# SunYangtian/UniGeo

Measured on AMD Instinct MI355X. Metric: frames/sec (384x512, 25-frame clip, 25 denoise steps), higher is better.
Workload: dtype fp16; 1 GPU; DepthCrafter SVD-UNet fp16, 25-step Euler, 25-frame 384x512 clips (BASELINE configs[1]); CLIP + VAE enc/dec + depth post-proc inside the timed region; one clip per ug_dc_run call, one call at a time (SURVEY 8d; reference eval.py:33-39); frames=25, height=384, width=512, denoise_steps=25, parallelism=clip-sharded x1, RCCL all_gather of depth, clips_in_flight_per_gpu=1, lanes=1

## Files before the change

### unigeo_amd/_lib.py

```python
import ctypes as C
import dataclasses
import json
import os
import warnings

import numpy as np

_HERE = os.path.dirname(os.path.abspath(__file__))
LIB_PATH = os.environ.get("UG_LIB_PATH") or os.path.join(_HERE, "csrc", "libunigeo_hip.so")

EXPORTS = [
    "ug_unet_config_default", "ug_vae_config_default", "ug_clip_config_default",
    "ug_create", "ug_destroy", "ug_last_error", "ug_workspace_peak",
    "ug_load_tensor", "ug_bind_unet", "ug_bind_vae", "ug_bind_clip",
    "ug_dc_set_inputs", "ug_dc_run", "ug_dc_run_windows", "ug_dc_get_outputs", "ug_dc_device_ptrs", "ug_dc_set_trace", "ug_dc_set_guidance", "ug_unet_forward_pair", "ug_dc_set_inputs_ex", "ug_dc_get_noise", "ug_op_philox_u32", "ug_op_randn", "ug_op_u8_to_frames", "ug_set_vae_encode_fp32", "ug_set_concurrency", "ug_set_coscheduled", "ug_set_fp8_linears", "ug_op_linear_mx8", "ug_set_ff_fused", "ug_op_ff", "ug_op_ln_ff", "ug_bench_ff", "ug_bench_flash", "ug_tune_flash", "ug_tune_ff",
    "ug_eval_depth", "ug_eval_normal", "ug_depth_eval_opts_default", "ug_eval_depth_ex", "ug_eval_depth_global", "ug_op_masked_median", "ug_eval_depth_l1_info", "ug_op_l1_fit", "ug_clip_embed", "ug_vae_encode", "ug_vae_decode", "ug_unet_forward", "ug_normals_from_depth",
    "ug_op_linear", "ug_op_conv", "ug_op_conv_gn", "ug_op_groupnorm", "ug_op_layernorm", "ug_op_flash_attn",
    "ug_op_temporal_attn", "ug_op_attention_generic", "ug_op_flash_attn_dh", "ug_op_euler_step", "ug_op_flash_cross_attn", "ug_op_temporal_attn_nv",
    "ug_op_groupnorm_ex", "ug_op_layernorm_ex",
    "ug_op_split_pair", "ug_op_gn32_pair", "ug_op_conv_wide", "ug_op_attn_wide",
    "ug_bind_stablenormal", "ug_sn_run", "ug_sn_unet_forward", "ug_sn_dino", "ug_sn_vae_decode", "ug_sn_vae_encode", "ug_resize_bilinear",
    "ug_pcd_opts_default", "ug_pcd_world_points", "ug_eval_pcd", "ug_op_pcd_nn", "ug_op_pcd_select", "ug_op_pcd_knn_normals", "ug_eval_pcd_fps", "ug_op_pcd_fps",
    "ug_eval_pcd_ex", "ug_op_pcd_nn_grid", "ug_op_pcd_knn_normals_grid",
    "ug_pointmap_opts_default", "ug_pointmap_focal", "ug_pointmap_poses",
    "ug_vis_depth_range", "ug_vis_panels", "ug_prep_resize_frames", "ug_prep_gt", "ug_prep_gt_ex",
    "ug_register_opts_default", "ug_prep_register_depth",
    "ug_profile_begin", "ug_profile_begin_shapes", "ug_profile_end", "ug_bench_gemm", "ug_bench_groupnorm", "ug_bench_mfma_peak", "ug_tune_force",
]


class UNetConfigC(C.Structure):
    _fields_ = [("in_channels", C.c_int), ("out_channels", C.c_int), ("num_levels", C.c_int),
                ("block_out_channels", C.c_int * 8), ("num_attention_heads", C.c_int * 8),
                ("down_has_attn", C.c_int * 8),
                ("layers_per_block", C.c_int), ("cross_attention_dim", C.c_int),
                ("addition_time_embed_dim", C.c_int), ("projection_class_embeddings_input_dim", C.c_int),
                ("norm_groups", C.c_int),
                ("eps_cross_attn_blocks", C.c_float), ("eps_plain_down_block", C.c_float),
                ("eps_mid_block", C.c_float), ("eps_up_blocks", C.c_float)]


class VAEConfigC(C.Structure):
# ... 100 lines not shown
    _set_argtypes(lib, {"ug_eval_pcd_fps": [vp, vp, vp, vp, C.c_long, C.c_long, C.POINTER(PcdOptsC), vp, vp, vp, vp, vp],
                        "ug_op_pcd_fps": [vp, vp, C.c_long, C.c_long, vp, vp]})
    _set_argtypes(lib, {"ug_eval_pcd_ex": [vp, vp, vp, vp, C.c_long, vp, C.c_long, C.POINTER(PcdOptsC), ip, vp, vp, vp, vp, vp, vp],
                        "ug_op_pcd_nn_grid": [vp, vp, C.c_long, vp, C.c_long, vp, vp, vp, vp],
                        "ug_op_pcd_knn_normals_grid": [vp, vp, C.c_long, ip, vp, vp, vp]})
    _set_argtypes(lib, {"ug_pointmap_opts_default": [C.POINTER(PointmapOptsC)],
                        "ug_pointmap_focal": [vp, vp, ip, ip, C.c_double, C.c_double, vp],
                        "ug_pointmap_poses": [vp, vp, vp, ip, ip, ip, C.c_double, C.c_double, C.c_double, C.POINTER(PointmapOptsC), vp, vp, vp, vp]})
    if hasattr(lib, "ug_pointmap_opts_default"):
        lib.ug_pointmap_opts_default.restype = None
    _set_argtypes(lib, {"ug_vis_depth_range": [vp, vp, C.c_long, vp],
                        "ug_vis_panels": [vp, vp, vp, vp, ip, ip, ip, ip, C.c_float, C.c_float, vp, vp, ip, vp]})
    _set_argtypes(lib, {"ug_prep_resize_frames": [vp, vp, ip, ip, ip, ip, ip, vp, vp, ip, vp, vp, ip, vp],
                        "ug_prep_gt": [vp, vp, C.c_float, vp, vp, vp, ip, ip, ip, vp, ip, vp, ip, C.c_float, vp, vp, vp, vp, vp],
                        "ug_prep_gt_ex": [vp, vp, C.c_float, vp, vp, vp, ip, ip, ip, vp, ip, vp, ip, C.c_float, vp, vp, vp, vp, vp, C.c_uint]})
    _set_argtypes(lib, {"ug_register_opts_default": [C.POINTER(RegisterOptsC)],
                        "ug_prep_register_depth": [vp, vp, ip, ip, ip, C.POINTER(RegisterOptsC), vp]})
    lib.ug_clip_embed.argtypes = [vp, vp, ip, ip, ip, vp]
    lib.ug_vae_encode.argtypes = [vp, vp, ip, ip, ip, vp]
    lib.ug_vae_decode.argtypes = [vp, vp, ip, ip, ip, vp]
    lib.ug_unet_forward.argtypes = [vp, vp, ip, ip, ip, C.c_float, vp, vp]
    lib.ug_normals_from_depth.argtypes = [vp, vp, vp, ip, ip, ip, vp]
    lib.ug_op_linear.argtypes = [vp, vp, ip, ip, vp, ip, vp, vp, C.c_float, C.c_float, ip, ip, vp]
    lib.ug_op_conv.argtypes = [vp, vp, ip, vp, ip, ip, ip, ip, vp, vp, ip, ip, ip, ip, ip, ip, ip, vp]
    lib.ug_op_groupnorm.argtypes = [vp, vp, ip, vp, ip, ip, ip, ip, C.c_float, ip, ip, vp, vp, vp]
    lib.ug_op_conv_gn.argtypes = [vp, vp, ip, ip, ip, ip, vp, vp, vp, ip, ip, ip, ip, C.c_float, ip, vp, vp, vp, vp, vp, vp]
    lib.ug_op_layernorm.argtypes = [vp, vp, ip, ip, C.c_float, vp, vp, vp, ip, vp, vp]
    lib.ug_op_flash_attn.argtypes = [vp, vp, ip, ip, ip, vp]
    lib.ug_op_temporal_attn.argtypes = [vp, vp, ip, ip, ip, vp]
    lib.ug_op_attention_generic.argtypes = [vp, vp, ip, ip, ip, ip, vp]
# ... 55 lines not shown
    c = VAEConfigC()
    c.in_channels, c.out_channels, c.latent_channels = cfg.in_channels, cfg.out_channels, cfg.latent_channels
    c.num_levels = len(cfg.block_out_channels)
    _fill8(c.block_out_channels, cfg.block_out_channels)
    c.layers_per_block, c.norm_groups, c.scaling_factor = cfg.layers_per_block, cfg.norm_groups, cfg.scaling_factor
    return c


def _clip_c(cfg):
    c = CLIPConfigC()
    c.hidden_size, c.intermediate_size = cfg.hidden_size, cfg.intermediate_size
    c.num_hidden_layers, c.num_attention_heads = cfg.num_hidden_layers, cfg.num_attention_heads
    c.image_size, c.patch_size, c.layer_norm_eps = cfg.image_size, cfg.patch_size, cfg.layer_norm_eps
    c.projection_dim = getattr(cfg, "projection_dim", 0)
    return c


class Engine:

    def __init__(self, device_id=0, workspace_bytes=2 << 30, persist_bytes=1 << 30):
        self.lib = load_library()
        self.ctx = self.lib.ug_create(int(device_id), int(workspace_bytes), int(persist_bytes))
        if not self.ctx:
            raise RuntimeError("ug_create failed: " + self.lib.ug_last_error(None).decode())
        self.device_id = device_id
        self.l1_info = None
        self._l1_warned = False

    def close(self):
        if getattr(self, "ctx", None):
# ... 762 lines not shown
        cv = conv or {}
        self._ck(self.lib.ug_bench_gemm(self.ctx, M, N, K, int(conv is not None), cv.get("T", 0), cv.get("H", 0), cv.get("W", 0),
                                        cv.get("C0", 0), cv.get("C1", 0), cv.get("kt", 1), cv.get("k", 1), cv.get("stride", 1),
                                        cv.get("ups", 1), cfg, split, iters, _ptr(out)))
        Mr, Kr = float(out[3]), float(out[4])
        return float(out[0]), 2.0 * Mr * N * Kr / (out[0] * 1e-3) / 1e12, int(out[1]), int(out[2])

    def bench_mfma_peak(self, iters=20000):
        out = np.zeros(1, np.float32)
        self._ck(self.lib.ug_bench_mfma_peak(self.ctx, int(iters), _ptr(out)))
        return float(out[0])

    def tune_force(self, cfg=-1, split=-1):
        self._ck(self.lib.ug_tune_force(self.ctx, int(cfg), int(split)))

    def bench_groupnorm(self, C0, C1, T, HW, temporal, mode, iters=20):
        out = np.zeros(1, np.float32)
        self._ck(self.lib.ug_bench_groupnorm(self.ctx, C0, C1, T, HW, int(temporal), mode, iters, _ptr(out)))
        return float(out[0])

    def profile_begin(self, shapes=False):
        self._ck((self.lib.ug_profile_begin_shapes if shapes else self.lib.ug_profile_begin)(self.ctx))

    def profile_end(self):
        prof = json.loads(self.lib.ug_profile_end(self.ctx).decode())
        self.last_profile_order = prof.pop("__order__", None)
        return prof

    def workspace_peak(self):
        return int(self.lib.ug_workspace_peak(self.ctx))
# ... 1 lines not shown
```

### unigeo_amd/csrc/common.h

```cpp
#pragma once
#include <hip/hip_runtime.h>
#include <hip/hip_fp16.h>
#include <stdint.h>
#include <stdio.h>
#include <stdexcept>
#include <string>

typedef _Float16 f16;
typedef _Float16 f16x2 __attribute__((ext_vector_type(2)));
typedef _Float16 f16x4 __attribute__((ext_vector_type(4)));
typedef _Float16 f16x8 __attribute__((ext_vector_type(8)));
typedef float f32x4 __attribute__((ext_vector_type(4)));
typedef float f32x16 __attribute__((ext_vector_type(16)));

#define UG_CHECK(expr)                                                                        \
  do {                                                                                        \
    hipError_t _e = (expr);                                                                   \
    if (_e != hipSuccess)                                                                     \
      throw std::runtime_error(std::string(#expr) + " failed: " + hipGetErrorString(_e) +    \
                               " at " + __FILE__ + ":" + std::to_string(__LINE__));           \
  } while (0)

#define UG_REQUIRE(cond, msg)                                                                 \
  do {                                                                                        \
    if (!(cond))                                                                              \
      throw std::runtime_error(std::string("requirement failed: ") + #cond + " : " + (msg) + \
                               " at " + __FILE__ + ":" + std::to_string(__LINE__));           \
  } while (0)

static inline int cdiv(long a, long b) { return (int)((a + b - 1) / b); }
static inline int ug_dev_slot() { int d = 0; (void)hipGetDevice(&d); return d & 31; }

enum { UG_ACT_NONE = 0, UG_ACT_SILU = 1, UG_ACT_GELU = 2 };
enum { UG_F_GEGLU = 1, UG_F_OUT_F32 = 2, UG_F_NOXCD = 4, UG_F_PRIO = 8 ,
       UG_F_XCDROUND = 32 ,
       UG_F_R1_F32 = 16  };

struct GemmP {
  const f16* A0; const f16* A1;
  int C0, C1;
  int M, N, K;
  int conv;
  int T, Hi, Wi, Ho, Wo;
  int ups, stride, pad_t, pad_l;
  int kt, ky, kx;
  const f16* W; long ldw;
  const f16* bias; const f16* bias2;
  const f16* R1; long ldr1; float c1;
  const f16* R2; long ldr2; float c2;
  float c0;
  void* Out; long ldo;
// ... 13 lines not shown
  int group_m;
  int halo_tw, halo_lg;
  int tune_cfg_p1, tune_split_p1, tune_knobs;
  float2* stat_part; int stat_hw;
};
struct GemmTune { int cfg = -1, split = -1, knobs = 0; };
static inline void gemm_apply_tune(GemmP& p, const GemmTune& t) { p.tune_cfg_p1 = t.cfg + 1; p.tune_split_p1 = t.split + 1; p.tune_knobs = t.knobs; }
void launch_gemm_mx8(const GemmP& p, hipStream_t s);
void launch_quant_mx8(const f16* x, long ldx, long M, int K, unsigned char* q, unsigned* scales, long ld_s, hipStream_t s);
void launch_gemm(const GemmP& p, int batch, hipStream_t s, int* stat_rb = nullptr);
bool gemm_stream_supported(const GemmP& p, int batch);
void launch_gemm_stream(const GemmP& p, hipStream_t s);
bool conv_halo_supported(const GemmP& p, int batch, int bm, int bn);
void launch_conv_halo(const GemmP& p, int bm, int bn, hipStream_t s);
void gemm_plan(const GemmP& p, int batch, int* cfg_out, int* split_out);

struct FFusedP {
  const f16* X; const f16* W1; const f16* b1; const f16* W2; const f16* b2;
  const f16* R1; const f16* R2; float c0, c1, c2;
  f16* Out; int M, C; const f16* zero;
  const f16* ln_g; const f16* ln_b; float ln_eps; const f16* addvec; int rows_per_vec;
  int variant;
};
bool ff_fused_supported(int C);
void launch_ff_fused(const FFusedP& p, hipStream_t s);

struct GroupNormP {
  const f16* X0; const f16* X1; int C0, C1;
  int T, HW, G; float eps; int temporal; int silu;
  const f16* gamma; const f16* beta;
// ... 227 lines not shown
```

### unigeo_amd/csrc/kernels/gemm.hip

```cpp
#include "../common.h"
#include <algorithm>

#include "gemm_common.h"

template <int BM, int BN, int BK, int NST, int WMW, int WNW> struct GemmOcc {
  static constexpr int lds = NST * (BM + BN) * BK * 2;
  static constexpr int wg_lds = (160 * 1024) / lds;
  static constexpr int wg = wg_lds < 1 ? 1 : (wg_lds > 4 ? 4 : wg_lds);
  static constexpr int wps_raw = wg * WMW * WNW / 4;
  static constexpr int wps = wps_raw < 1 ? 1 : (wps_raw > 4 ? 4 : wps_raw);
};

#ifdef UG_GEMM_TRACE
#define UG_STAMP(slot)                                                                                   \
  do {                                                                                                   \
    if (traced && fi >= 8 && fi < 32) {                                                                  \
      unsigned long long c_;                                                                             \
      asm volatile("s_memtime %0\n\ts_waitcnt lgkmcnt(0)" : "=s"(c_)::"memory");                         \
      if (lane == 0) tr_lds[(fi - 8) * 5 + (slot)] = (unsigned)c_;                                       \
    }                                                                                                    \
  } while (0)
#else
#define UG_STAMP(slot) do {} while (0)
#endif
// ... 21 lines not shown
  const int wm = wave / WNW, wn = wave % WNW;
  if (NWAVE == 8 && wave >= 4 && ((BM == 256 && BN == 256) || (p.flags & UG_F_PRIO))) __builtin_amdgcn_s_setprio(1);
  const int ntn = (p.N + BN - 1) / BN, ntm = (p.M + BM - 1) / BM;
  const int ntiles = ntm * ntn;

  const int bz = blockIdx.z;
  const int bo = bz / p.nb_inner, bi = bz - bo * p.nb_inner;
  const f16* A0 = p.A0 + bo * p.sA_o + bi * p.sA_i;
  const f16* Wb = p.W + bo * p.sW_o + bi * p.sW_i;
  const long out_off = bo * p.sO_o + bi * p.sO_i;

  const int pc = lane % CPR;
  const int lrow = lane / CPR;
  const int Cin = p.C0 + p.C1;

  const int nk_all = (p.K + BK - 1) / BK;
  int kt_lo = 0, kt_hi = nk_all;
  if (p.splitk > 1) {
    const int per = (nk_all + p.splitk - 1) / p.splitk;
    kt_lo = min(nk_all, (int)blockIdx.y * per);
    kt_hi = min(nk_all, kt_lo + per);
  }
  const int nk = max(kt_hi - kt_lo, 1);

  const int nwg = gridDim.x, w = blockIdx.x;
  const TileWalk tw = tile_walk(p.flags, ntiles, nwg, w);
  const int my_tiles = tw.count;
  const int total_it = my_tiles * nk;

  int a_lc[AI]; bool a_ok[AI]; const f16* a_ptr[AI]; int a_t[AI], a_y[AI], a_x[AI];
  int a_pix[AI]; unsigned a_mask[AI];
  const bool fastconv = CONV && UNI;
  int a_par[AI];
  int b_lc[BI]; const f16* b_ptr[BI]; bool b_ok[BI];
  unsigned a_off[AI], a_off1[AI], b_off[BI];
  const int cshift = CONV ? ((p.kt >> 1) * p.Hi + p.pad_t) * p.Wi + p.pad_l : 0;
  __amdgpu_buffer_rsrc_t rA0, rA1, rW;
  if (BUFA) {
    rA0 = __builtin_amdgcn_make_buffer_rsrc((void*)(A0 - (long)cshift * p.C0), 0, (int)SENT, 0x00020000);
    rA1 = __builtin_amdgcn_make_buffer_rsrc((void*)((CONV && p.A1) ? p.A1 - (long)cshift * p.C1 : A0), 0, (int)SENT, 0x00020000);
    rW = __builtin_amdgcn_make_buffer_rsrc((void*)Wb, 0, (int)SENT, 0x00020000);
  }
// ... 252 lines not shown
    if (traced && fi == 40) {
      __builtin_amdgcn_s_waitcnt(0);
      for (int i = lane; i < 24 * 5; i += 64) ((unsigned*)p.trace)[(wave == 4 ? 24 * 5 : 0) + i] = tr_lds[i];
    }
#endif
    if (++cp_ks != nk) continue;
    cp_ks = 0;
    const int ti = cp_ti++;

    drain = true;
    const int tile = tw.first + ti * tw.step;
    { int etm, etn; tile_coord_p(p, tile, ntm, ntn, etm, etn);
      if constexpr (ST) tile_epilogue_stats<MT, NT, WTM, WTN>(p, acc, etm * BM, etn * BN, wm, wn, lane, etm * WMW + wm);
      else if constexpr (BM * BN < 65536) {
        if (lean_epi == 1) tile_epilogue_lean<MT, NT, WTM, WTN, false>(p, acc, etm * BM, etn * BN, wm, wn, lane, out_off, nullptr);
        else if constexpr (NT == 4 && !CONV) { if (lean_epi == 2) tile_epilogue_geglu_lean<MT, NT, WTM, WTN>(p, acc, etm * BM, etn * BN, wm, wn, lane, out_off); else tile_epilogue<MT, NT, WTM, WTN>(p, acc, etm * BM, etn * BN, wm, wn, lane, out_off); }
        else tile_epilogue<MT, NT, WTM, WTN>(p, acc, etm * BM, etn * BN, wm, wn, lane, out_off);
      } else if constexpr (NT == 4 && !CONV) { if (lean_epi == 2) tile_epilogue_geglu_lean<MT, NT, WTM, WTN>(p, acc, etm * BM, etn * BN, wm, wn, lane, out_off); else tile_epilogue<MT, NT, WTM, WTN>(p, acc, etm * BM, etn * BN, wm, wn, lane, out_off); }
      else tile_epilogue<MT, NT, WTM, WTN>(p, acc, etm * BM, etn * BN, wm, wn, lane, out_off); }
  }
}

template <int BM, int BN, int NST, int WMW, int WNW, bool CONV, bool ST = false>
__global__ __launch_bounds__(512, 2) void gemm_ldr_kernel(const GemmP p) {
  constexpr int BK = 64;
  static_assert(WMW * WNW == 8, "two waves per SIMD");
  constexpr unsigned SENT = 0x80000000u;
  constexpr int WTM = BM / WMW, WTN = BN / WNW;
  constexpr int MT = WTM / 16, NT = WTN / 16;
  constexpr int WID = 4 * NT;
  constexpr int AI = BM / 64, BI = BN / 64;
  constexpr int LA = 2 * AI, LB = 2 * BI;
  constexpr int STAGE = (BM + BN) * BK;
  static_assert(AI >= 1 && BI >= 1 && NST >= 2 && NST <= 3, "tile / ring");
// ... 4 lines not shown
  const int wave = __builtin_amdgcn_readfirstlane(tid >> 6);
  const int wm = wave / WNW, wn = wave % WNW;
  const bool loader = wave >= 4;
  const int ntn = (p.N + BN - 1) / BN, ntm = (p.M + BM - 1) / BM;
  const int ntiles = ntm * ntn;

  const int bz = blockIdx.z;
  const int bo = bz / p.nb_inner, bi = bz - bo * p.nb_inner;
  const f16* A0 = p.A0 + bo * p.sA_o + bi * p.sA_i;
  const f16* Wb = p.W + bo * p.sW_o + bi * p.sW_i;
  const long out_off = bo * p.sO_o + bi * p.sO_i;

  const int pc = lane & 7, lrow = lane >> 3;
  const int Cin = p.C0 + p.C1;

  const int nk_all = (p.K + BK - 1) / BK;
  int kt_lo = 0, kt_hi = nk_all;
  if (p.splitk > 1) {
    const int per = (nk_all + p.splitk - 1) / p.splitk;
    kt_lo = min(nk_all, (int)blockIdx.y * per);
    kt_hi = min(nk_all, kt_lo + per);
  }
  const int nk = max(kt_hi - kt_lo, 1);

  const int nwg = gridDim.x, w = blockIdx.x;
  const TileWalk tw = tile_walk(p.flags, ntiles, nwg, w);
  const int my_tiles = tw.count;
  const int total_it = my_tiles * nk;

  unsigned a_st[LA], b_off[LB];
  const int lc16_0 = (pc ^ ((0 + (lrow >> 1)) & 7)) * 16, lc16_1 = (pc ^ ((4 + (lrow >> 1)) & 7)) * 16;
  const int cshift = CONV ? ((p.kt >> 1) * p.Hi + p.pad_t) * p.Wi + p.pad_l : 0;
  const __amdgpu_buffer_rsrc_t rA0 = __builtin_amdgcn_make_buffer_rsrc((void*)(A0 - (long)cshift * p.C0), 0, (int)SENT, 0x00020000);
  const __amdgpu_buffer_rsrc_t rA1 =
      __builtin_amdgcn_make_buffer_rsrc((void*)((CONV && p.A1) ? p.A1 - (long)cshift * p.C1 : A0), 0, (int)SENT, 0x00020000);
  const __amdgpu_buffer_rsrc_t rW = __builtin_amdgcn_make_buffer_rsrc((void*)Wb, 0, (int)SENT, 0x00020000);

  auto setup_tile = [&](int tile) {
    int tm, tn; tile_coord_p(p, tile, ntm, ntn, tm, tn);
    const int m0 = tm * BM, n0 = tn * BN;
#pragma unroll
    for (int l = 0; l < LA; ++l) {
// ... 144 lines not shown
    }
#ifdef UG_GEMM_TRACE
    if (traced && fi == 40) {
      __builtin_amdgcn_s_waitcnt(0);
      for (int i = lane; i < 24 * 5; i += 64) ((unsigned*)p.trace)[(wave == 4 ? 24 * 5 : 0) + i] = tr_lds[i];
    }
#endif
    if (++cp_ks != nk) continue;
    cp_ks = 0;
    const int tile = tw.first + (cp_ti++) * tw.step;
    drain = true;
    { int etm, etn; tile_coord_p(p, tile, ntm, ntn, etm, etn);
      if constexpr (ST) tile_epilogue_stats<MT, NT, WTM, WTN>(p, acc, etm * BM, etn * BN, wm, wn, lane, etm * WMW + wm);
      else if constexpr (BM * BN < 65536) {
        if (lean_epi == 1) tile_epilogue_lean<MT, NT, WTM, WTN, false>(p, acc, etm * BM, etn * BN, wm, wn, lane, out_off, nullptr);
        else if constexpr (NT == 4 && !CONV) { if (lean_epi == 2) tile_epilogue_geglu_lean<MT, NT, WTM, WTN>(p, acc, etm * BM, etn * BN, wm, wn, lane, out_off); else tile_epilogue<MT, NT, WTM, WTN>(p, acc, etm * BM, etn * BN, wm, wn, lane, out_off); }
        else tile_epilogue<MT, NT, WTM, WTN>(p, acc, etm * BM, etn * BN, wm, wn, lane, out_off);
      } else if constexpr (NT == 4 && !CONV) { if (lean_epi == 2) tile_epilogue_geglu_lean<MT, NT, WTM, WTN>(p, acc, etm * BM, etn * BN, wm, wn, lane, out_off); else tile_epilogue<MT, NT, WTM, WTN>(p, acc, etm * BM, etn * BN, wm, wn, lane, out_off); }
      else tile_epilogue<MT, NT, WTM, WTN>(p, acc, etm * BM, etn * BN, wm, wn, lane, out_off); }
  }
}

static bool gemm_can_bufa(const GemmP& p, int BK, bool packed) {
  const long lim = (1L << 31) - 64;
  if ((long)p.N * p.ldw * 2 >= lim) return false;
  if (p.conv) {
    const bool kc_ok = p.kchunk || p.kt * p.ky * p.kx == 1 || (p.C0 + p.C1) == BK;
    const bool uni = kc_ok && ((p.C0 + p.C1) % BK) == 0 && (p.C0 % BK) == 0 && p.kt * p.ky * p.kx <= (packed ? 9 : 32);
    const long px = (long)p.T * p.Hi * p.Wi + ((long)(p.kt >> 1) * p.Hi + p.pad_t) * p.Wi + p.pad_l + 1;
    return uni && p.ups == 1 && px * p.C0 * 2 < lim && px * p.C1 * 2 < lim && (!packed || px < (1L << 23));
  }
  return p.K % BK == 0 && (long)p.M * p.C0 * 2 < lim;
}

// ... 17 lines not shown
  constexpr int STAGE = (BM + BN) * BK;
  extern __shared__ __attribute__((aligned(16))) f16 smem[];

  const int tid = threadIdx.x, lane = tid & 63;
  const int wave = __builtin_amdgcn_readfirstlane(tid >> 6);
  const bool producer = wave >= NCW;
  const int ntn = (p.N + BN - 1) / BN, ntm = (p.M + BM - 1) / BM;
  const int ntiles = ntm * ntn;

  const int bz = blockIdx.z;
  const int bo = bz / p.nb_inner, bi = bz - bo * p.nb_inner;
  const f16* A0 = p.A0 + bo * p.sA_o + bi * p.sA_i;
  const f16* Wb = p.W + bo * p.sW_o + bi * p.sW_i;
  const long out_off = bo * p.sO_o + bi * p.sO_i;

  const int nk_all = (p.K + BK - 1) / BK;
  int kt_lo = 0, kt_hi = nk_all;
  if (p.splitk > 1) {
    const int per = (nk_all + p.splitk - 1) / p.splitk;
    kt_lo = min(nk_all, (int)blockIdx.y * per);
    kt_hi = min(nk_all, kt_lo + per);
  }
  const int nk = max(kt_hi - kt_lo, 1);

  const int nwg = gridDim.x, w = blockIdx.x;
  const TileWalk tw = tile_walk(p.flags, ntiles, nwg, w);
  const int my_tiles = tw.count;
  const int total_it = my_tiles * nk;

  if (producer) {
    const int pw = wave - NCW;
    const int pc = lane & 7, lrow = lane >> 3;
    const int Cin = p.C0 + p.C1;
    const int lc16_0 = (pc ^ ((0 + (lrow >> 1)) & 7)) * 16, lc16_1 = (pc ^ ((4 + (lrow >> 1)) & 7)) * 16;
    const int cshift = CONV ? ((p.kt >> 1) * p.Hi + p.pad_t) * p.Wi + p.pad_l : 0;
    const __amdgpu_buffer_rsrc_t rA0 = __builtin_amdgcn_make_buffer_rsrc((void*)(A0 - (long)cshift * p.C0), 0, (int)SENT, 0x00020000);
    const __amdgpu_buffer_rsrc_t rA1 =
        __builtin_amdgcn_make_buffer_rsrc((void*)((CONV && p.A1) ? p.A1 - (long)cshift * p.C1 : A0), 0, (int)SENT, 0x00020000);
    const __amdgpu_buffer_rsrc_t rW = __builtin_amdgcn_make_buffer_rsrc((void*)Wb, 0, (int)SENT, 0x00020000);
    unsigned a_st[LA], b_off[LB];
    int ld_ti = 0, ld_ks = 0, ld_slot = 0;
    int u_it = 0, u_iy = 0, u_ix = 0, u_cb = 0;
// ... 184 lines not shown
    }
    UG_STAMP(1);
    asm volatile("s_waitcnt lgkmcnt(0)" ::: "memory");
    UG_STAMP(2);
    __builtin_amdgcn_s_barrier();
    asm volatile("" ::: "memory");
    UG_STAMP(3);
    if (++cp_ks == nk) {
      cp_ks = 0;
      const int tile = tw.first + (cp_ti++) * tw.step;
      { int etm, etn; tile_coord_p(p, tile, ntm, ntn, etm, etn);
        if constexpr (ST) tile_epilogue_stats<MT, NT, WTM, WTN>(p, acc, etm * BM, etn * BN, wm, wn, lane, etm * WMW + wm);
        else if (PREK && do_pre) {
          if (lean) tile_epilogue_lean<MT, NT, WTM, WTN, PREK>(p, acc, etm * BM, etn * BN, wm, wn, lane, out_off, &pre);
          else if constexpr (NT == 4) { if (lean_geglu) tile_epilogue_geglu_lean<MT, NT, WTM, WTN>(p, acc, etm * BM, etn * BN, wm, wn, lane, out_off);
            else tile_epilogue<MT, NT, WTM, WTN, PREK>(p, acc, etm * BM, etn * BN, wm, wn, lane, out_off, &pre); }
          else tile_epilogue<MT, NT, WTM, WTN, PREK>(p, acc, etm * BM, etn * BN, wm, wn, lane, out_off, &pre);
        } else if constexpr (PREK) {
          tile_epilogue<MT, NT, WTM, WTN>(p, acc, etm * BM, etn * BN, wm, wn, lane, out_off);
        } else {
          if (lean) tile_epilogue_lean<MT, NT, WTM, WTN, false>(p, acc, etm * BM, etn * BN, wm, wn, lane, out_off, nullptr);
          else if constexpr (NT == 4) { if (lean_geglu) tile_epilogue_geglu_lean<MT, NT, WTM, WTN>(p, acc, etm * BM, etn * BN, wm, wn, lane, out_off);
            else tile_epilogue<MT, NT, WTM, WTN>(p, acc, etm * BM, etn * BN, wm, wn, lane, out_off); }
          else tile_epilogue<MT, NT, WTM, WTN>(p, acc, etm * BM, etn * BN, wm, wn, lane, out_off);
        } }
    }
#ifdef UG_GEMM_TRACE
    if (traced && fi == 40) {
      __builtin_amdgcn_s_waitcnt(0);
      for (int i = lane; i < 24 * 5; i += 64) ((unsigned*)p.trace)[(wave == 4 ? 24 * 5 : 0) + i] = tr_lds[i];
    }
#endif
  }
}

template <int BN, int WMW, int WNW, int BM = 256>
static void launch_ws(const GemmP& p, int batch, hipStream_t s) {
  const int ntiles = cdiv(p.M, BM) * cdiv(p.N, BN);
#ifdef UG_GEMM_TRACE
  const size_t lds = ws_nst(BM, BN) * (BM + BN) * 64 * sizeof(f16) + 2048;
#else
  const size_t lds = ws_nst(BM, BN) * (BM + BN) * 64 * sizeof(f16);
#endif
  static bool attr[32] = {};
  bool& at = attr[ug_dev_slot()];
  if (!at) {
    UG_CHECK(hipFuncSetAttribute((const void*)gemm_ws_kernel<BM, BN, WMW, WNW, true>, hipFuncAttributeMaxDynamicSharedMemorySize, (int)lds));
    UG_CHECK(hipFuncSetAttribute((const void*)gemm_ws_kernel<BM, BN, WMW, WNW, false>, hipFuncAttributeMaxDynamicSharedMemorySize, (int)lds));
    at = true;
  }
  const int split = p.splitk > 1 ? p.splitk : 1;
  int gx = std::max(8, 256 / (split * batch));
  gx = (gx / 8) * 8;
  gx = std::min(gx, ntiles);
  dim3 grid(gx, split, batch);
  if (p.stat_part) {
    if constexpr (BN == 128) {
      UG_REQUIRE(p.conv, "producer / consumer kernel: epilogue statistics for convolutions only");
      static bool attrs[32] = {};
      bool& ats = attrs[ug_dev_slot()];
      if (!ats) { UG_CHECK(hipFuncSetAttribute((const void*)gemm_ws_kernel<BM, BN, WMW, WNW, true, true>, hipFuncAttributeMaxDynamicSharedMemorySize, (int)lds)); ats = true; }
      hipLaunchKernelGGL((gemm_ws_kernel<BM, BN, WMW, WNW, true, true>), grid, dim3((WMW * WNW + 4) * 64), lds, s, p);
      return;
    } else UG_REQUIRE(false, "producer / consumer kernel: epilogue statistics on 128-column tiles only");
  }
  if (p.conv) hipLaunchKernelGGL((gemm_ws_kernel<BM, BN, WMW, WNW, true>), grid, dim3((WMW * WNW + 4) * 64), lds, s, p);
  else hipLaunchKernelGGL((gemm_ws_kernel<BM, BN, WMW, WNW, false>), grid, dim3((WMW * WNW + 4) * 64), lds, s, p);
}

template <int BM, int BN, int NST, int WMW, int WNW>
static void launch_ldr(const GemmP& p, int batch, hipStream_t s) {
  UG_REQUIRE(p.m_off == 0, "row-split launches need the producer / consumer kernel");
  const int ntiles = cdiv(p.M, BM) * cdiv(p.N, BN);
#ifdef UG_GEMM_TRACE
  const size_t lds = (size_t)NST * (BM + BN) * 64 * sizeof(f16) + 1024;
#else
  const size_t lds = (size_t)NST * (BM + BN) * 64 * sizeof(f16);
#endif
  static bool attr[32] = {};
  bool& at = attr[ug_dev_slot()];
  if (!at) {
    UG_CHECK(hipFuncSetAttribute((const void*)gemm_ldr_kernel<BM, BN, NST, WMW, WNW, true>, hipFuncAttributeMaxDynamicSharedMemorySize, (int)lds));
    UG_CHECK(hipFuncSetAttribute((const void*)gemm_ldr_kernel<BM, BN, NST, WMW, WNW, false>, hipFuncAttributeMaxDynamicSharedMemorySize, (int)lds));
    at = true;
  }
  const int per_cu = (160 * 1024) / (int)lds < 1 ? 1 : std::min(2, (160 * 1024) / (int)lds);
  const int split = p.splitk > 1 ? p.splitk : 1;
  int gx = std::max(8, (per_cu * 256) / (split * batch));
  gx = (gx / 8) * 8;
  gx = std::min(gx, ntiles);
  dim3 grid(gx, split, batch);
  if (p.stat_part) {
    if constexpr (BM == 256 && BN == 256) {
      UG_REQUIRE(p.conv, "loader kernel: epilogue statistics for convolutions only");
      static bool attrs[32] = {};
      bool& ats = attrs[ug_dev_slot()];
      if (!ats) { UG_CHECK(hipFuncSetAttribute((const void*)gemm_ldr_kernel<BM, BN, NST, WMW, WNW, true, true>, hipFuncAttributeMaxDynamicSharedMemorySize, (int)lds)); ats = true; }
      hipLaunchKernelGGL((gemm_ldr_kernel<BM, BN, NST, WMW, WNW, true, true>), grid, dim3(512), lds, s, p);
      return;
    } else UG_REQUIRE(false, "loader kernel: epilogue statistics on the 256 x 256 tile only");
  }
  if (p.conv) hipLaunchKernelGGL((gemm_ldr_kernel<BM, BN, NST, WMW, WNW, true>), grid, dim3(512), lds, s, p);
  else hipLaunchKernelGGL((gemm_ldr_kernel<BM, BN, NST, WMW, WNW, false>), grid, dim3(512), lds, s, p);
}

__global__ __launch_bounds__(256) void splitk_epilogue(const GemmP p) {
// ... 24 lines not shown
    if (p.act == UG_ACT_SILU) {
#pragma unroll
      for (int q = 0; q < 8; ++q) v[q] = silu_f(v[q]);
    } else if (p.act == UG_ACT_GELU) {
#pragma unroll
      for (int q = 0; q < 8; ++q) v[q] = gelu_f(v[q]);
    }
    f16x8 h;
#pragma unroll
    for (int q = 0; q < 8; ++q) h[q] = (f16)v[q];
    *(f16x8*)((f16*)p.Out + m * p.ldo + n) = h;
  }
}

template <int BM, int BN, int BK, int NST, int WMW, int WNW, bool CONV, bool UNI, bool BUFA = false, bool ST = false>
static void launch_t(const GemmP& p, int batch, hipStream_t s) {
  const int ntiles = cdiv(p.M, BM) * cdiv(p.N, BN);
#ifdef UG_GEMM_TRACE
  const size_t lds = (size_t)NST * (BM + BN) * BK * sizeof(f16) + 1024;
#else
  const size_t lds = (size_t)NST * (BM + BN) * BK * sizeof(f16);
#endif
  auto kern = gemm_kernel<BM, BN, BK, NST, WMW, WNW, CONV, UNI, BUFA, false, ST>;
  static bool attr[32] = {};
  bool& at = attr[ug_dev_slot()];
  if (!at) {
    if (lds > 64 * 1024) UG_CHECK(hipFuncSetAttribute((const void*)kern, hipFuncAttributeMaxDynamicSharedMemorySize, (int)lds));
    at = true;
  }
  const int per_cu = GemmOcc<BM, BN, BK, NST, WMW, WNW>::wg;
  const int split = p.splitk > 1 ? p.splitk : 1;
  const int cap = std::max(8, (per_cu * 256) / (split * batch));
  int gx = (cap / 8) * 8;
  gx = std::min(gx, ntiles);
  if (gx < ntiles && cap >= ntiles) gx = ntiles;
  if (p.tune_knobs & 1) gx = ntiles;
  dim3 grid(gx, split, batch);
  hipLaunchKernelGGL(kern, grid, dim3(WMW * WNW * 64), lds, s, p);
}

template <int BM, int BN, int BK, int NST, int WMW, int WNW>
static void launch_mode(const GemmP& p, int batch, hipStream_t s) {
  UG_REQUIRE(p.m_off == 0, "row-split launches need the producer / consumer kernel");
  const long lim = (1L << 31) - 64;
  const bool bufw = (long)p.N * p.ldw * 2 < lim && !(p.tune_knobs & 4);
  if (p.conv) {
    const bool kc_ok = p.kchunk || p.kt * p.ky * p.kx == 1 || (p.C0 + p.C1) == BK;
    const bool uni = kc_ok && ((p.C0 + p.C1) % BK) == 0 && (p.C0 % BK) == 0 && p.kt * p.ky * p.kx <= 32;
    const long px = (long)p.T * p.Hi * p.Wi + ((long)(p.kt >> 1) * p.Hi + p.pad_t) * p.Wi + p.pad_l + 1;
    const bool bufa = bufw && uni && p.ups == 1 && px * p.C0 * 2 < lim && px * p.C1 * 2 < lim;
    if (p.stat_part) {
      if constexpr ((BM == 256 && BN == 64 && NST == 2 && WMW == 4) || (BM == 256 && BN == 128 && NST == 3 && WMW == 2)) { UG_REQUIRE(uni && bufa, "statistics epilogue: buffer-addressed im2col only"); launch_t<BM, BN, BK, NST, WMW, WNW, true, true, true, true>(p, batch, s); return; }
// ... 351 lines not shown
```

### unigeo_amd/csrc/kernels/gemm_common.h

```cpp
#pragma once
#include "../common.h"
#include <type_traits>

typedef const __attribute__((address_space(1))) void* gptr_t;
typedef __attribute__((address_space(3))) void* lptr_t;

__device__ __forceinline__ float erf_as(float x) {
  const float ax = fabsf(x);
  const float t = __frcp_rn(1.0f + 0.3275911f * ax);
  const float y = ((((1.061405429f * t - 1.453152027f) * t + 1.421413741f) * t - 0.284496736f) * t + 0.254829592f) * t;
  const float r = 1.0f - y * __expf(-ax * ax);
  return copysignf(r, x);
}
__device__ __forceinline__ float gelu_f(float x) { return 0.5f * x * (1.0f + erf_as(x * 0.70710678118654752f)); }
__device__ __forceinline__ float silu_f(float x) { return x * __builtin_amdgcn_rcpf(1.0f + __expf(-x)); }

typedef float f32x2 __attribute__((ext_vector_type(2)));
__device__ __forceinline__ f32x2 geglu2(f32x2 h, f32x2 g) {
  const f32x2 ag = {__builtin_fabsf(g.x), __builtin_fabsf(g.y)};
  const f32x2 u = ag * 0.23164189f + 1.0f;
  const f32x2 t = {__builtin_amdgcn_rcpf(u.x), __builtin_amdgcn_rcpf(u.y)};
  f32x2 y = t * 0.5307027145f - 0.7265760135f;
  y = y * t + 0.7107068705f;
  y = y * t - 0.142248368f;
// ... 24 lines not shown
  tile_coord(tile, ntm, ntn, p.group_m, tm, tn);
  if (p.tm_T) { const int q = tm / p.tm_T; tm = (tm - q * p.tm_T) * p.tm_nb + q; }
}

struct TileWalk { int first, step, count; };
__device__ __forceinline__ TileWalk tile_walk(int flags, int ntiles, int nwg, int w) {
  TileWalk t;
  if (nwg % 8 != 0 || (flags & UG_F_NOXCD)) { t.first = w; t.step = nwg; t.count = (ntiles - w + nwg - 1) / nwg; return t; }
  const int x = w & 7, j = w >> 3, npx = nwg >> 3;
  if (flags & UG_F_XCDROUND) { t.first = x * npx + j; t.step = nwg; t.count = (ntiles - t.first + nwg - 1) / nwg; return t; }
  const int lo = (int)(((long)x * ntiles) >> 3), hi = (int)(((long)(x + 1) * ntiles) >> 3);
  t.first = lo + j; t.step = npx; t.count = max(0, (hi - lo - j + npx - 1) / npx);
  return t;
}

template <int N> struct HVec;
template <> struct HVec<8> { typedef f16x8 type; };
template <> struct HVec<4> { typedef f16x4 type; };

template <int MT, int NT> struct EpiPre {
  static constexpr int WID = 4 * NT, CH = (WID % 8 == 0) ? 8 : 4, NV = WID / CH;
  typedef typename HVec<CH>::type hvec;
  hvec b1[NV], b2[NV];
  hvec r1[MT][NV];
};
template <int MT, int NT, int WTM, int WTN>
__device__ __forceinline__ void epi_pre_cols(const GemmP& p, int n0, int wn, int lane, EpiPre<MT, NT>& pre) {
  typedef EpiPre<MT, NT> P;
  typedef typename P::hvec hvec;
  const int g = lane >> 4;
// ... 20 lines not shown
  if (nb + P::WID > p.N) return;
  if (epi_pre_r1_ok(p)) {
#pragma unroll
    for (int i = 0; i < MT; ++i) {
      const int m = m0 + wm * WTM + i * 16 + l15;
      if (m < p.M) {
#pragma unroll
        for (int v = 0; v < P::NV; ++v) pre.r1[i][v] = *(const hvec*)(p.R1 + (long)m * p.ldr1 + nb + v * P::CH);
      }
    }
  }
}

template <int MT, int NT, int WTM, int WTN, bool PRE = false>
__device__ __forceinline__ void tile_epilogue(const GemmP& p, f32x4 (&acc)[MT][NT], int m0, int n0, int wm, int wn, int lane,
                                              long out_off, const EpiPre<MT, NT>* pre = nullptr) {
  constexpr int WID = 4 * NT;
  constexpr int CH = (WID % 8 == 0) ? 8 : 4;
  typedef typename HVec<CH>::type hvec;
  const int l15 = lane & 15, g = lane >> 4;
  const bool geglu = (p.flags & UG_F_GEGLU) != 0;
  const bool of32 = (p.flags & UG_F_OUT_F32) != 0;
  const int Nout = geglu ? p.N / 2 : p.N;
  const int OW = geglu ? WID / 2 : WID;
  const int nb = n0 + wn * WTN + g * WID;
  if (p.splitk > 1) {
    float* P = p.partial + ((long)blockIdx.y * p.M) * p.N;
#pragma unroll
    for (int i = 0; i < MT; ++i) {
      const int m = m0 + wm * WTM + i * 16 + l15;
#pragma unroll
      for (int j = 0; j < NT; ++j) {
        const int n = nb + j * 4;
        if (m < p.M && n + 4 <= p.N) *(f32x4*)(P + (long)m * p.N + n) = acc[i][j];
        acc[i][j] = (f32x4){0.f, 0.f, 0.f, 0.f};
      }
    }
    return;
  }
  const int ob = geglu ? nb / 2 : nb;
  const bool full = (nb + WID <= p.N);
  const bool vec = full && ((p.ldo & 7) == 0) && (!p.R1 || (p.ldr1 & 7) == 0) &&
// ... 339 lines not shown
```

Before: 27.60 frames/s.

## Add XCD-aware panel tile mapping for GEMM launches with large weights

Adds a panel dispatch mode where each workgroup handles exactly one (tile, split-k slice), with N-column panels partitioned across the 8 XCDs so each XCD's L2 keeps a contiguous slice of the weight matrix. It turns on for single-batch GEMMs whose weight exceeds about 3 MB and whose grid fits in one wave, and it replaces the persistent tile walk and blockIdx.y split indexing. The goal is less weight re-fetching across XCD L2 caches. In exchange, persistence is lost, some padded workgroups exit idle, and the mapping only pays off if cross-XCD weight traffic was actually a bottleneck.

```diff
diff --git a/unigeo_amd/_lib.py b/unigeo_amd/_lib.py
--- a/unigeo_amd/_lib.py
+++ b/unigeo_amd/_lib.py
@@ -26,6 +26,7 @@
     "ug_vis_depth_range", "ug_vis_panels", "ug_prep_resize_frames", "ug_prep_gt", "ug_prep_gt_ex",
     "ug_register_opts_default", "ug_prep_register_depth",
     "ug_profile_begin", "ug_profile_begin_shapes", "ug_profile_end", "ug_bench_gemm", "ug_bench_groupnorm", "ug_bench_mfma_peak", "ug_tune_force",
+    "ug_op_panel_map", "ug_gemm_panel_launches",
 ]
 
 
@@ -156,6 +157,9 @@
     _set_argtypes(lib, {"ug_prep_resize_frames": [vp, vp, ip, ip, ip, ip, ip, vp, vp, ip, vp, vp, ip, vp],
                         "ug_prep_gt": [vp, vp, C.c_float, vp, vp, vp, ip, ip, ip, vp, ip, vp, ip, C.c_float, vp, vp, vp, vp, vp],
                         "ug_prep_gt_ex": [vp, vp, C.c_float, vp, vp, vp, ip, ip, ip, vp, ip, vp, ip, C.c_float, vp, vp, vp, vp, vp, C.c_uint]})
+    _set_argtypes(lib, {"ug_op_panel_map": [ip, ip, ip, vp, vp, ip], "ug_gemm_panel_launches": []})
+    if hasattr(lib, "ug_gemm_panel_launches"):
+        lib.ug_gemm_panel_launches.restype = C.c_long
     _set_argtypes(lib, {"ug_register_opts_default": [C.POINTER(RegisterOptsC)],
                         "ug_prep_register_depth": [vp, vp, ip, ip, ip, C.POINTER(RegisterOptsC), vp]})
     lib.ug_clip_embed.argtypes = [vp, vp, ip, ip, ip, vp]
@@ -241,6 +245,16 @@
     c.image_size, c.patch_size, c.layer_norm_eps = cfg.image_size, cfg.patch_size, cfg.layer_norm_eps
     c.projection_dim = getattr(cfg, "projection_dim", 0)
     return c
+
+
+def panel_map(ntm, ntn, splits):
+    lib = load_library()
+    n = lib.ug_op_panel_map(int(ntm), int(ntn), int(splits), None, None, 0)
+    if n < 0:
+        raise ValueError("panel_map: ntm, ntn, splits >= 1")
+    tiles, slices = np.empty(n, np.int32), np.empty(n, np.int32)
+    assert lib.ug_op_panel_map(int(ntm), int(ntn), int(splits), _ptr(tiles), _ptr(slices), n) == n
+    return tiles, slices
 
 
 class Engine:
@@ -1033,6 +1047,9 @@
     def tune_force(self, cfg=-1, split=-1):
         self._ck(self.lib.ug_tune_force(self.ctx, int(cfg), int(split)))
 
+    def panel_launches(self):
+        return int(self.lib.ug_gemm_panel_launches())
+
     def bench_groupnorm(self, C0, C1, T, HW, temporal, mode, iters=20):
         out = np.zeros(1, np.float32)
         self._ck(self.lib.ug_bench_groupnorm(self.ctx, C0, C1, T, HW, int(temporal), mode, iters, _ptr(out)))
diff --git a/unigeo_amd/csrc/common.h b/unigeo_amd/csrc/common.h
--- a/unigeo_amd/csrc/common.h
+++ b/unigeo_amd/csrc/common.h
@@ -34,7 +34,8 @@
 enum { UG_ACT_NONE = 0, UG_ACT_SILU = 1, UG_ACT_GELU = 2 };
 enum { UG_F_GEGLU = 1, UG_F_OUT_F32 = 2, UG_F_NOXCD = 4, UG_F_PRIO = 8 ,
        UG_F_XCDROUND = 32 ,
-       UG_F_R1_F32 = 16  };
+       UG_F_R1_F32 = 16 ,
+       UG_F_PANEL = 64  };
 
 struct GemmP {
   const f16* A0; const f16* A1;
@@ -78,6 +79,8 @@
 bool conv_halo_supported(const GemmP& p, int batch, int bm, int bn);
 void launch_conv_halo(const GemmP& p, int bm, int bn, hipStream_t s);
 void gemm_plan(const GemmP& p, int batch, int* cfg_out, int* split_out);
+int gemm_panel_map_host(int ntm, int ntn, int splits, int* tiles, int* slices, int cap);
+long gemm_panel_launches();
 
 struct FFusedP {
   const f16* X; const f16* W1; const f16* b1; const f16* W2; const f16* b2;
diff --git a/unigeo_amd/csrc/kernels/gemm.hip b/unigeo_amd/csrc/kernels/gemm.hip
--- a/unigeo_amd/csrc/kernels/gemm.hip
+++ b/unigeo_amd/csrc/kernels/gemm.hip
@@ -1,5 +1,6 @@
 #include "../common.h"
 #include <algorithm>
+#include <atomic>
 
 #include "gemm_common.h"
 
@@ -59,18 +60,23 @@
   const int lrow = lane / CPR;
   const int Cin = p.C0 + p.C1;
 
+  const int nwg = gridDim.x, w = blockIdx.x;
+  TileWalk tw; int ks = blockIdx.y;
+  if (p.flags & UG_F_PANEL) {
+    const PanelSlot ps = panel_slot(ntm, ntn, max(p.splitk, 1), w);
+    if (ps.tile < 0) return;
+    tw.first = ps.tile; tw.step = 0; tw.count = 1; ks = ps.slice;
+  } else tw = tile_walk(p.flags, ntiles, nwg, w);
+  const int my_tiles = tw.count;
+
   const int nk_all = (p.K + BK - 1) / BK;
   int kt_lo = 0, kt_hi = nk_all;
   if (p.splitk > 1) {
     const int per = (nk_all + p.splitk - 1) / p.splitk;
-    kt_lo = min(nk_all, (int)blockIdx.y * per);
+    kt_lo = min(nk_all, ks * per);
     kt_hi = min(nk_all, kt_lo + per);
   }
   const int nk = max(kt_hi - kt_lo, 1);
-
-  const int nwg = gridDim.x, w = blockIdx.x;
-  const TileWalk tw = tile_walk(p.flags, ntiles, nwg, w);
-  const int my_tiles = tw.count;
   const int total_it = my_tiles * nk;
 
   int a_lc[AI]; bool a_ok[AI]; const f16* a_ptr[AI]; int a_t[AI], a_y[AI], a_x[AI];
@@ -353,10 +359,10 @@
       if constexpr (ST) tile_epilogue_stats<MT, NT, WTM, WTN>(p, acc, etm * BM, etn * BN, wm, wn, lane, etm * WMW + wm);
       else if constexpr (BM * BN < 65536) {
         if (lean_epi == 1) tile_epilogue_lean<MT, NT, WTM, WTN, false>(p, acc, etm * BM, etn * BN, wm, wn, lane, out_off, nullptr);
-        else if constexpr (NT == 4 && !CONV) { if (lean_epi == 2) tile_epilogue_geglu_lean<MT, NT, WTM, WTN>(p, acc, etm * BM, etn * BN, wm, wn, lane, out_off); else tile_epilogue<MT, NT, WTM, WTN>(p, acc, etm * BM, etn * BN, wm, wn, lane, out_off); }
-        else tile_epilogue<MT, NT, WTM, WTN>(p, acc, etm * BM, etn * BN, wm, wn, lane, out_off);
-      } else if constexpr (NT == 4 && !CONV) { if (lean_epi == 2) tile_epilogue_geglu_lean<MT, NT, WTM, WTN>(p, acc, etm * BM, etn * BN, wm, wn, lane, out_off); else tile_epilogue<MT, NT, WTM, WTN>(p, acc, etm * BM, etn * BN, wm, wn, lane, out_off); }
-      else tile_epilogue<MT, NT, WTM, WTN>(p, acc, etm * BM, etn * BN, wm, wn, lane, out_off); }
+        else if constexpr (NT == 4 && !CONV) { if (lean_epi == 2) tile_epilogue_geglu_lean<MT, NT, WTM, WTN>(p, acc, etm * BM, etn * BN, wm, wn, lane, out_off); else tile_epilogue<MT, NT, WTM, WTN>(p, acc, etm * BM, etn * BN, wm, wn, lane, out_off, nullptr, ks); }
+        else tile_epilogue<MT, NT, WTM, WTN>(p, acc, etm * BM, etn * BN, wm, wn, lane, out_off, nullptr, ks);
+      } else if constexpr (NT == 4 && !CONV) { if (lean_epi == 2) tile_epilogue_geglu_lean<MT, NT, WTM, WTN>(p, acc, etm * BM, etn * BN, wm, wn, lane, out_off); else tile_epilogue<MT, NT, WTM, WTN>(p, acc, etm * BM, etn * BN, wm, wn, lane, out_off, nullptr, ks); }
+      else tile_epilogue<MT, NT, WTM, WTN>(p, acc, etm * BM, etn * BN, wm, wn, lane, out_off, nullptr, ks); }
   }
 }
 
@@ -391,18 +397,23 @@
   const int pc = lane & 7, lrow = lane >> 3;
   const int Cin = p.C0 + p.C1;
 
+  const int nwg = gridDim.x, w = blockIdx.x;
+  TileWalk tw; int ks = blockIdx.y;
+  if (p.flags & UG_F_PANEL) {
+    const PanelSlot ps = panel_slot(ntm, ntn, max(p.splitk, 1), w);
+    if (ps.tile < 0) return;
+    tw.first = ps.tile; tw.step = 0; tw.count = 1; ks = ps.slice;
+  } else tw = tile_walk(p.flags, ntiles, nwg, w);
+  const int my_tiles = tw.count;
+
   const int nk_all = (p.K + BK - 1) / BK;
   int kt_lo = 0, kt_hi = nk_all;
   if (p.splitk > 1) {
     const int per = (nk_all + p.splitk - 1) / p.splitk;
-    kt_lo = min(nk_all, (int)blockIdx.y * per);
+    kt_lo = min(nk_all, ks * per);
     kt_hi = min(nk_all, kt_lo + per);
   }
   const int nk = max(kt_hi - kt_lo, 1);
-
-  const int nwg = gridDim.x, w = blockIdx.x;
-  const TileWalk tw = tile_walk(p.flags, ntiles, nwg, w);
-  const int my_tiles = tw.count;
   const int total_it = my_tiles * nk;
 
   unsigned a_st[LA], b_off[LB];
@@ -577,10 +588,10 @@
       if constexpr (ST) tile_epilogue_stats<MT, NT, WTM, WTN>(p, acc, etm * BM, etn * BN, wm, wn, lane, etm * WMW + wm);
       else if constexpr (BM * BN < 65536) {
         if (lean_epi == 1) tile_epilogue_lean<MT, NT, WTM, WTN, false>(p, acc, etm * BM, etn * BN, wm, wn, lane, out_off, nullptr);
-        else if constexpr (NT == 4 && !CONV) { if (lean_epi == 2) tile_epilogue_geglu_lean<MT, NT, WTM, WTN>(p, acc, etm * BM, etn * BN, wm, wn, lane, out_off); else tile_epilogue<MT, NT, WTM, WTN>(p, acc, etm * BM, etn * BN, wm, wn, lane, out_off); }
-        else tile_epilogue<MT, NT, WTM, WTN>(p, acc, etm * BM, etn * BN, wm, wn, lane, out_off);
-      } else if constexpr (NT == 4 && !CONV) { if (lean_epi == 2) tile_epilogue_geglu_lean<MT, NT, WTM, WTN>(p, acc, etm * BM, etn * BN, wm, wn, lane, out_off); else tile_epilogue<MT, NT, WTM, WTN>(p, acc, etm * BM, etn * BN, wm, wn, lane, out_off); }
-      else tile_epilogue<MT, NT, WTM, WTN>(p, acc, etm * BM, etn * BN, wm, wn, lane, out_off); }
+        else if constexpr (NT == 4 && !CONV) { if (lean_epi == 2) tile_epilogue_geglu_lean<MT, NT, WTM, WTN>(p, acc, etm * BM, etn * BN, wm, wn, lane, out_off); else tile_epilogue<MT, NT, WTM, WTN>(p, acc, etm * BM, etn * BN, wm, wn, lane, out_off, nullptr, ks); }
+        else tile_epilogue<MT, NT, WTM, WTN>(p, acc, etm * BM, etn * BN, wm, wn, lane, out_off, nullptr, ks);
+      } else if constexpr (NT == 4 && !CONV) { if (lean_epi == 2) tile_epilogue_geglu_lean<MT, NT, WTM, WTN>(p, acc, etm * BM, etn * BN, wm, wn, lane, out_off); else tile_epilogue<MT, NT, WTM, WTN>(p, acc, etm * BM, etn * BN, wm, wn, lane, out_off, nullptr, ks); }
+      else tile_epilogue<MT, NT, WTM, WTN>(p, acc, etm * BM, etn * BN, wm, wn, lane, out_off, nullptr, ks); }
   }
 }
 
@@ -628,18 +639,23 @@
   const f16* Wb = p.W + bo * p.sW_o + bi * p.sW_i;
   const long out_off = bo * p.sO_o + bi * p.sO_i;
 
+  const int nwg = gridDim.x, w = blockIdx.x;
+  TileWalk tw; int ks = blockIdx.y;
+  if (p.flags & UG_F_PANEL) {
+    const PanelSlot ps = panel_slot(ntm, ntn, max(p.splitk, 1), w);
+    if (ps.tile < 0) return;
+    tw.first = ps.tile; tw.step = 0; tw.count = 1; ks = ps.slice;
+  } else tw = tile_walk(p.flags, ntiles, nwg, w);
+  const int my_tiles = tw.count;
+
   const int nk_all = (p.K + BK - 1) / BK;
   int kt_lo = 0, kt_hi = nk_all;
   if (p.splitk > 1) {
     const int per = (nk_all + p.splitk - 1) / p.splitk;
-    kt_lo = min(nk_all, (int)blockIdx.y * per);
+    kt_lo = min(nk_all, ks * per);
     kt_hi = min(nk_all, kt_lo + per);
   }
   const int nk = max(kt_hi - kt_lo, 1);
-
-  const int nwg = gridDim.x, w = blockIdx.x;
-  const TileWalk tw = tile_walk(p.flags, ntiles, nwg, w);
-  const int my_tiles = tw.count;
   const int total_it = my_tiles * nk;
 
   if (producer) {
@@ -854,15 +870,15 @@
         else if (PREK && do_pre) {
           if (lean) tile_epilogue_lean<MT, NT, WTM, WTN, PREK>(p, acc, etm * BM, etn * BN, wm, wn, lane, out_off, &pre);
           else if constexpr (NT == 4) { if (lean_geglu) tile_epilogue_geglu_lean<MT, NT, WTM, WTN>(p, acc, etm * BM, etn * BN, wm, wn, lane, out_off);
-            else tile_epilogue<MT, NT, WTM, WTN, PREK>(p, acc, etm * BM, etn * BN, wm, wn, lane, out_off, &pre); }
-          else tile_epilogue<MT, NT, WTM, WTN, PREK>(p, acc, etm * BM, etn * BN, wm, wn, lane, out_off, &pre);
+            else tile_epilogue<MT, NT, WTM, WTN, PREK>(p, acc, etm * BM, etn * BN, wm, wn, lane, out_off, &pre, ks); }
+          else tile_epilogue<MT, NT, WTM, WTN, PREK>(p, acc, etm * BM, etn * BN, wm, wn, lane, out_off, &pre, ks);
         } else if constexpr (PREK) {
-          tile_epilogue<MT, NT, WTM, WTN>(p, acc, etm * BM, etn * BN, wm, wn, lane, out_off);
+          tile_epilogue<MT, NT, WTM, WTN>(p, acc, etm * BM, etn * BN, wm, wn, lane, out_off, nullptr, ks);
         } else {
           if (lean) tile_epilogue_lean<MT, NT, WTM, WTN, false>(p, acc, etm * BM, etn * BN, wm, wn, lane, out_off, nullptr);
           else if constexpr (NT == 4) { if (lean_geglu) tile_epilogue_geglu_lean<MT, NT, WTM, WTN>(p, acc, etm * BM, etn * BN, wm, wn, lane, out_off);
-            else tile_epilogue<MT, NT, WTM, WTN>(p, acc, etm * BM, etn * BN, wm, wn, lane, out_off); }
-          else tile_epilogue<MT, NT, WTM, WTN>(p, acc, etm * BM, etn * BN, wm, wn, lane, out_off);
+            else tile_epilogue<MT, NT, WTM, WTN>(p, acc, etm * BM, etn * BN, wm, wn, lane, out_off, nullptr, ks); }
+          else tile_epilogue<MT, NT, WTM, WTN>(p, acc, etm * BM, etn * BN, wm, wn, lane, out_off, nullptr, ks);
         } }
     }
 #ifdef UG_GEMM_TRACE
@@ -874,8 +890,29 @@
   }
 }
 
+static std::atomic<long> g_panel_launches{0};
+long gemm_panel_launches() { return g_panel_launches.load(); }
+int gemm_panel_map_host(int ntm, int ntn, int splits, int* tiles, int* slices, int cap) {
+  const int n = panel_grid(ntm, ntn, splits);
+  for (int b = 0; b < n && b < cap; ++b) { const PanelSlot ps = panel_slot(ntm, ntn, splits, b); tiles[b] = ps.tile; slices[b] = ps.slice; }
+  return n;
+}
+static int panel_dispatch(GemmP& p, int batch, int bm, int bn, int per_cu) {
+  if ((p.tune_knobs & (33554432 | 1 | 2 | 128)) || batch != 1 || p.m_off != 0) return 0;
+  const int ntm = cdiv(p.M, bm), ntn = cdiv(p.N, bn), split = p.splitk > 1 ? p.splitk : 1;
+  if (ntm < 2) return 0;
+  const long P = ((long)ntn * split + 7) / 8;
+  if (8 * P * ntm > (long)per_cu * 256 || P * ntm > (long)per_cu * 32) return 0;
+  if (!(p.tune_knobs & 67108864) && (double)p.N * p.K * 2.0 <= 3.0 * (1 << 20)) return 0;
+  p.flags |= UG_F_PANEL; p.group_m = 1; p.tm_T = p.tm_nb = 0;
+  g_panel_launches.fetch_add(1, std::memory_order_relaxed);
+  return (int)(8 * P * ntm);
+}
+
 template <int BN, int WMW, int WNW, int BM = 256>
-static void launch_ws(const GemmP& p, int batch, hipStream_t s) {
+static void launch_ws(const GemmP& p0, int batch, hipStream_t s) {
+  GemmP p = p0;
+  const int panel = panel_dispatch(p, batch, BM, BN, 1);
   const int ntiles = cdiv(p.M, BM) * cdiv(p.N, BN);
 #ifdef UG_GEMM_TRACE
   const size_t lds = ws_nst(BM, BN) * (BM + BN) * 64 * sizeof(f16) + 2048;
@@ -893,7 +930,7 @@
   int gx = std::max(8, 256 / (split * batch));
   gx = (gx / 8) * 8;
   gx = std::min(gx, ntiles);
-  dim3 grid(gx, split, batch);
+  const dim3 grid = panel ? dim3(panel, 1, 1) : dim3(gx, split, batch);
   if (p.stat_part) {
     if constexpr (BN == 128) {
       UG_REQUIRE(p.conv, "producer / consumer kernel: epilogue statistics for convolutions only");
@@ -909,7 +946,8 @@
 }
 
 template <int BM, int BN, int NST, int WMW, int WNW>
-static void launch_ldr(const GemmP& p, int batch, hipStream_t s) {
+static void launch_ldr(const GemmP& p0, int batch, hipStream_t s) {
+  GemmP p = p0;
   UG_REQUIRE(p.m_off == 0, "row-split launches need the producer / consumer kernel");
   const int ntiles = cdiv(p.M, BM) * cdiv(p.N, BN);
 #ifdef UG_GEMM_TRACE
@@ -929,7 +967,8 @@
   int gx = std::max(8, (per_cu * 256) / (split * batch));
   gx = (gx / 8) * 8;
   gx = std::min(gx, ntiles);
-  dim3 grid(gx, split, batch);
+  const int panel = panel_dispatch(p, batch, BM, BN, per_cu);
+  const dim3 grid = panel ? dim3(panel, 1, 1) : dim3(gx, split, batch);
   if (p.stat_part) {
     if constexpr (BM == 256 && BN == 256) {
       UG_REQUIRE(p.conv, "loader kernel: epilogue statistics for convolutions only");
@@ -984,7 +1023,8 @@
 }
 
 template <int BM, int BN, int BK, int NST, int WMW, int WNW, bool CONV, bool UNI, bool BUFA = false, bool ST = false>
-static void launch_t(const GemmP& p, int batch, hipStream_t s) {
+static void launch_t(const GemmP& p0, int batch, hipStream_t s) {
+  GemmP p = p0;
   const int ntiles = cdiv(p.M, BM) * cdiv(p.N, BN);
 #ifdef UG_GEMM_TRACE
   const size_t lds = (size_t)NST * (BM + BN) * BK * sizeof(f16) + 1024;
@@ -1005,7 +1045,8 @@
   gx = std::min(gx, ntiles);
   if (gx < ntiles && cap >= ntiles) gx = ntiles;
   if (p.tune_knobs & 1) gx = ntiles;
-  dim3 grid(gx, split, batch);
+  const int panel = panel_dispatch(p, batch, BM, BN, per_cu);
+  const dim3 grid = panel ? dim3(panel, 1, 1) : dim3(gx, split, batch);
   hipLaunchKernelGGL(kern, grid, dim3(WMW * WNW * 64), lds, s, p);
 }
 
diff --git a/unigeo_amd/csrc/kernels/gemm_common.h b/unigeo_amd/csrc/kernels/gemm_common.h
--- a/unigeo_amd/csrc/kernels/gemm_common.h
+++ b/unigeo_amd/csrc/kernels/gemm_common.h
@@ -62,6 +62,19 @@
   return t;
 }
 
+struct PanelSlot { int tile, slice; };
+__host__ __device__ __forceinline__ int panel_grid(int ntm, int ntn, int S) { return 8 * ((ntn * S + 7) / 8) * ntm; }
+__host__ __device__ __forceinline__ PanelSlot panel_slot(int ntm, int ntn, int S, int b) {
+  const int np = ntn * S, g = b & 7, j = b >> 3;
+  const int lo = (g * np) >> 3, hi = ((g + 1) * np) >> 3;
+  const int i = j / ntm, tm = j - i * ntm, q = lo + i;
+  PanelSlot r;
+  if (q >= hi) { r.tile = -1; r.slice = 0; return r; }
+  r.slice = q / ntn;
+  r.tile = tm * ntn + (q - r.slice * ntn);
+  return r;
+}
+
 template <int N> struct HVec;
 template <> struct HVec<8> { typedef f16x8 type; };
 template <> struct HVec<4> { typedef f16x4 type; };
@@ -112,7 +125,7 @@
 
 template <int MT, int NT, int WTM, int WTN, bool PRE = false>
 __device__ __forceinline__ void tile_epilogue(const GemmP& p, f32x4 (&acc)[MT][NT], int m0, int n0, int wm, int wn, int lane,
-                                              long out_off, const EpiPre<MT, NT>* pre = nullptr) {
+                                              long out_off, const EpiPre<MT, NT>* pre = nullptr, int ks = (int)blockIdx.y) {
   constexpr int WID = 4 * NT;
   constexpr int CH = (WID % 8 == 0) ? 8 : 4;
   typedef typename HVec<CH>::type hvec;
@@ -123,7 +136,7 @@
   const int OW = geglu ? WID / 2 : WID;
   const int nb = n0 + wn * WTN + g * WID;
   if (p.splitk > 1) {
-    float* P = p.partial + ((long)blockIdx.y * p.M) * p.N;
+    float* P = p.partial + ((long)ks * p.M) * p.N;
 #pragma unroll
     for (int i = 0; i < MT; ++i) {
       const int m = m0 + wm * WTM + i * 16 + l15;
```

New measurement: 27.59 frames/s. About the same (-0.0%).
